# byungsook/deep-fluids

Measured on AMD Instinct MI355X. Metric: velocity-field voxels/sec (3D 64x96x64 train step), whole job; per-GPU in `per_gpu`, higher is better.
Workload: dtype f32; 1 GPU; cfg3: 3D smoke3 64x96x64 (Z,Y,X) fp32, GeneratorBE3 filters=128 num_conv=4, per-GPU batch 16, full train step (fwd+curl3+jacobian3+L1 losses+bwd+Adam); global_batch=16, batch_per_gpu=16, params=7483523, parallelism=dp1

## Files before the change

deep_fluids_amd/_lib.py:

```python
import ctypes
import os
import re

_HERE = os.path.dirname(os.path.abspath(__file__))
LIB_PATH = os.path.join(_HERE, "csrc", "libdeepfluids_hip.so")
TUNING_LIB_PATH = os.path.join(_HERE, "csrc", "libdeepfluids_hip_tuning.so")
HEADER_PATH = os.path.join(os.path.dirname(_HERE), "include", "deepfluids_hip.h")

P, I64, I32, F32 = ctypes.c_void_p, ctypes.c_int64, ctypes.c_int, ctypes.c_float

SIGNATURES = {
    "df_version": (I32, []),
    "df_last_error": (ctypes.c_char_p, []),
    "df_curl2d_fwd": (I32, [P, P, I64, I64, I64, P]),
    "df_curl2d_bwd": (I32, [P, P, I64, I64, I64, P]),
    "df_jacobian2d_fwd": (I32, [P, P, P, I64, I64, I64, P]),
    "df_jacobian2d_bwd": (I32, [P, P, P, I64, I64, I64, P]),
    "df_jacobian3d_fwd": (I32, [P, P, P, I64, I64, I64, I64, P]),
    "df_jacobian3d_bwd": (I32, [P, P, P, I64, I64, I64, I64, P]),
    "df_divergence2d": (I32, [P, P, I64, I64, I64, P]),
    "df_divergence3d": (I32, [P, P, I64, I64, I64, I64, P]),
    "df_velocity_loss3d_workspace_bytes": (I64, [I64, I64, I64, I64]),
    "df_velocity_loss3d_fwd": (I32, [P, P, P, P, P, I64, I64, I64, I64, P, I64, P]),
    "df_velocity_loss3d_bwd": (I32, [P, P, P, P, P, I64, I64, I64, I64, P, I64, P]),
# ... 21 lines not shown
    "df_concat2_fwd": (I32, [P, P, P, I64, I64, I64, P]),
    "df_concat2_bwd": (I32, [P, P, P, I64, I64, I64, P]),
    "df_dilate2_odd": (I32, [P, P, I64, I64, I64, I64, I64, I32, P]),
    "df_kl_bernoulli_fwd": (I32, [P, I64, I64, I64, F32, P, P]),
    "df_kl_bernoulli_bwd": (I32, [P, P, F32, P, I64, I64, I64, F32, P]),
    "df_sigmoid_fwd": (I32, [P, P, I64, P]),
    "df_sigmoid_bwd": (I32, [P, P, P, I64, P]),
    "df_mse_mean_fwd": (I32, [P, P, I64, P, P, I64, P]),
    "df_mse_mean_bwd": (I32, [P, P, P, F32, P, I64, P]),
    "df_colsum_workspace_bytes": (I64, [I64, I64]),
    "df_colsum": (I32, [P, P, I64, I64, P, I64, P]),
    "df_adam_tf1_step": (I32, [P, P, P, P, I64, F32, F32, F32, F32, F32, P]),
    "df_conv_packed_elems": (I64, [I64, I64, I64, I32]),
    "df_conv_pack_weights": (I32, [P, P, I64, I64, I64, I32, P]),
    "df_conv_fwd": (I32, [P, P, P, P, P, P, I64, I64, I64, I64, I64, I64, I32, I32, F32, P]),
    "df_conv_s2_fwd": (I32, [P, P, P, P, I64, I64, I64, I64, I64, I64, I32, I32, F32, P]),
    "df_conv_s2_wgrad_workspace_bytes": (I64, [I64, I64, I64, I64, I64, I64, I32]),
    "df_conv_s2_wgrad": (I32, [P, P, P, P, I64, I64, I64, I64, I64, I64, I32, P, I64, P]),
    "df_conv_s2_dgrad": (I32, [P, P, P, I64, I64, I64, I64, I64, I64, I32, P]),
    "df_conv_s2_dgrad_form": (I32, [P, I64, I64]),
    "df_upconv_packed_elems": (I64, [I64, I64, I32, I32]),
    "df_upconv_pack_weights": (I32, [P, P, I64, I64, I32, I32, P]),
    "df_upconv_fwd": (I32, [P, P, P, P, I64, I64, I64, I64, I64, I64, I32, I32, F32, P]),
    "df_upconv_dgrad": (I32, [P, P, P, I64, I64, I64, I64, I64, I64, I32, P]),
    "df_upconv_wgrad_workspace_bytes": (I64, [I64, I64, I64, I64, I64, I64, I32]),
    "df_upconv_wgrad": (I32, [P, P, P, P, I64, I64, I64, I64, I64, I64, I32, P, I64, P]),
    "df_add_up2x": (I32, [P, P, P, I64, I64, I64, I64, I64, I32, P]),
    "df_wino_packed_elems": (I64, [I64, I64, I32]),
    "df_wino_pack_weights": (I32, [P, P, I64, I64, I32, P]),
    "df_wino_conv_fwd": (I32, [P, P, P, P, P, P, I64, I64, I64, I64, I64, I64, I32, F32, P]),
    "df_wino_conv_fwd_addup": (I32, [P, P, P, P, P, P, I64, I64, I64, I64, I64, I64, F32, P]),
    "df_wino_conv_fwd_addup_bits": (I32, [P, P, P, P, P, P, I64, I64, I64, I64, I64, I64, F32, P]),
    "df_lrelu_bits_bwd_pool2x": (I32, [P, P, P, P, F32, I64, I64, I64, I64, I64, P]),
    "df_wino_upconv_fwd": (I32, [P, P, P, P, I64, I64, I64, I64, I64, I64, I32, F32, P]),
    "df_wino_upconv_dgrad": (I32, [P, P, P, I64, I64, I64, I64, I64, I64, P]),
    "df_wino_signbits_bytes": (I64, [I64, I64, I64, I64, I64]),
    "df_wino_conv_fwd_bits": (I32, [P, P, P, P, P, P, I64, I64, I64, I64, I64, I64, I32, F32, P]),
    "df_wino_upconv_fwd_bits": (I32, [P, P, P, P, P, I64, I64, I64, I64, I64, I64, F32, P]),
    "df_wino43_packed_elems": (I64, [I64, I64, I32]),
    "df_wino43_pack_weights": (I32, [P, P, I64, I64, I32, P]),
    "df_wino43_conv": (I32, [P, P, P, P, P, P, P, P, P, I64, I64, I64, I64, I64, I64, I32, F32, P]),
    "df_wino2d43_packed_elems": (I64, [I64, I64, I32]),
    "df_wino2d43_pack_weights": (I32, [P, P, I64, I64, I32, P]),
    "df_wino2d43_conv": (I32, [P, P, P, P, P, P, I64, I64, I64, I64, I64, I32, F32, P]),
    "df_wino2d43_signbits_bytes": (I64, [I64, I64, I64, I64]),
    "df_wino2d43_conv_bits": (I32, [P, P, P, P, P, P, I64, I64, I64, I64, I64, I32, F32, P]),
    "df_wino2d43_conv_addup_bits": (I32, [P, P, P, P, P, P, I64, I64, I64, I64, I64, F32, P]),
    "df_lrelu_words2d_bwd_pool2x": (I32, [P, P, P, P, F32, I64, I64, I64, I64, P]),
    "df_wino2d_packed_elems": (I64, [I64, I64, I32]),
    "df_wino2d_pack_weights": (I32, [P, P, I64, I64, I32, P]),
    "df_wino2d_conv_fwd": (I32, [P, P, P, P, P, P, I64, I64, I64, I64, I64, I32, F32, P]),
    "df_wino2d_upconv_fwd": (I32, [P, P, P, P, I64, I64, I64, I64, I64, I32, F32, P]),
    "df_wino2d_upconv_dgrad": (I32, [P, P, P, I64, I64, I64, I64, I64, P]),
    "df_conv_packed_elems_bf16x3": (I64, [I64, I64, I64, I32]),
    "df_conv_pack_weights_bf16x3": (I32, [P, P, I64, I64, I64, I32, P]),
    "df_conv_fwd_bf16x3": (I32, [P, P, P, P, P, P, I64, I64, I64, I64, I64, I64, I32, I32, F32, P]),
    "df_upconv_packed_elems_bf16x3": (I64, [I64, I64, I32, I32]),
    "df_upconv_pack_weights_bf16x3": (I32, [P, P, I64, I64, I32, I32, P]),
    "df_upconv_fwd_bf16x3": (I32, [P, P, P, P, I64, I64, I64, I64, I64, I64, I32, I32, F32, P]),
    "df_upconv_dgrad_bf16x3": (I32, [P, P, P, I64, I64, I64, I64, I64, I64, I32, P]),
    "df_conv_wgrad_bf16x3": (I32, [P, P, P, P, I64, I64, I64, I64, I64, I64, I32, P, I64, P]),
    "df_upconv_wgrad_bf16x3": (I32, [P, P, P, P, I64, I64, I64, I64, I64, I64, I32, P, I64, P]),
    "df_adam_tf1_step_dev": (I32, [P, P, P, P, I64, P, F32, F32, F32, P]),
    "df_gd_step": (I32, [P, P, I64, F32, F32, P]),
    "df_gd_step_dev": (I32, [P, P, I64, P, P]),
    "df_store_scalars": (I32, [P, I64, F32, F32, F32, F32, P]),
# ... 164 lines not shown
```

deep_fluids_amd/csrc/conv_small.hip:

```cpp
#include "conv_args.hpp"

namespace dfconv {
namespace {

using df::ceil_div;
typedef float f32x2 __attribute__((ext_vector_type(2)));

template <int KZ, int TZ, int TY, int TX, int CO, bool VEC>
__global__ __launch_bounds__(kThreads) void conv_small_n_kernel(const ConvArgs a) {
  static_assert(TZ * TY * TX == kThreads, "one thread per output voxel");
  constexpr int PZ = KZ / 2;
  constexpr int HZ = TZ + KZ - 1, HY = TY + 2, HX = TX + 2, HV = HZ * HY * HX;
  constexpr int NPIECE = HV * (CK / 4);
  constexpr int NLOAD = (NPIECE + kThreads - 1) / kThreads;
  constexpr int NTAP = KZ * 9;
  constexpr int S4 = LDS_STRIDE / 4;
  __shared__ __attribute__((aligned(16))) float sA[HV * LDS_STRIDE];
  __shared__ __attribute__((aligned(16))) f32x4 sWt[NTAP * 4 * 4];
  const f32x4* sA4 = reinterpret_cast<const f32x4*>(sA);

  const int tid = threadIdx.x;
  const int tile = xcd_tile(blockIdx.x, a.ntiles);
  const int ix = tile % a.nx;
  int t2 = tile / a.nx;
// ... 342 lines not shown
  t.RS = a.W * a.Cin + 8;
  const size_t lds = static_cast<size_t>(4) * 19 * t.RS * sizeof(float);
  const int wps = a.Cout == 128 ? 2 : 1;
  int ns = 4 / wps * df::kCUs;
  if (ns > t.nrows) ns = t.nrows / 2 * 2;
  t.rows_per = (t.nrows + ns - 1) / ns;
  t.flags = a.flags; t.leak = a.leak;
  dim3 grid((unsigned)ceil_div(ceil_div(t.nrows, t.rows_per) * wps, 4));
  const bool two = a.W * a.Cin > 256;
#define DF_TK2(CI, COV, NPV)                                                                                                                \
  do {                                                                                                                                      \
    if (lds > 64 * 1024)                                                                                                                    \
      if (hipError_t e = hipFuncSetAttribute(reinterpret_cast<const void*>(&conv_thin_k_mfma_kernel<CI, COV, NPV>),                         \
                                             hipFuncAttributeMaxDynamicSharedMemorySize, (int)lds))                                         \
        return df::fail((int)e, "df_conv_fwd(thin-K mfma): dynamic LDS opt-in: %s", hipGetErrorString(e));                                  \
    hipLaunchKernelGGL((conv_thin_k_mfma_kernel<CI, COV, NPV>), grid, dim3(kThreads), lds, s, t);                                           \
  } while (0)
#define DF_TK(CI)                                                                                                                           \
  do {                                                                                                                                      \
    if (a.Cout == 128) { if (two) DF_TK2(CI, 128, 2); else DF_TK2(CI, 128, 1); }                                                            \
    else { if (two) DF_TK2(CI, 64, 2); else DF_TK2(CI, 64, 1); }                                                                            \
  } while (0)
  switch (a.Cin) {
    case 1: DF_TK(1); break;
    case 2: DF_TK(2); break;
    case 3: DF_TK(3); break;
    default: DF_TK(4); break;
  }
#undef DF_TK
#undef DF_TK2
  return df::launched("df_conv_fwd(thin-K mfma)");
}

struct ThinNArgs {
  const float* x;
  const f32x4* wp;
  const float* bias;
  float* y;
  int B, D, H, W;
  int K8, Npad;
  int nsplit, rows_per;
  int flags;
  float leak;
};

template <int CO, int CIN>
__global__ __launch_bounds__(kThreads, 1) void conv_thin_n_mfma_kernel(const ThinNArgs a) {
  constexpr int NC = 9 * CO;
  constexpr int QN = CIN / 8;
  constexpr int NIT = 3 * QN;
  extern __shared__ __attribute__((aligned(16))) float smem_thin_n[];
  const int lane = threadIdx.x & 63;
  const int wave = __builtin_amdgcn_readfirstlane(threadIdx.x >> 6);
  const int stream = xcd_tile(blockIdx.x, gridDim.x) * 4 + wave;
  const int W = a.W, H = a.H, RS = W * CO + 8;
  float* ring = smem_thin_n + wave * 3 * RS;
  const int plane = stream / a.nsplit, part = stream % a.nsplit;
  if (plane >= a.B * a.D) return;
  const int y0 = part * a.rows_per;
  int y1 = y0 + a.rows_per;
  if (y1 > H) y1 = H;
  if (y0 >= y1) return;
  const int z = plane % a.D, b = plane / a.D;
  for (int i = lane; i < 3 * RS; i += 64) ring[i] = 0.f;
  const int n = lane & 31, kk = lane >> 5;

// ... 136 lines not shown
    default: DF_TN(3); break;
  }
#undef DF_TN
  return df::launched("df_conv_fwd(thin-N mfma)");
}

template <int KZ, int TZ, int TY, int TX>
int launch_small_k_t(ConvArgs a, hipStream_t s) {
  a.nz = (int)ceil_div(a.D, TZ); a.ny = (int)ceil_div(a.H, TY); a.nx = (int)ceil_div(a.W, TX);
  const int64_t nt = static_cast<int64_t>(a.B) * a.nz * a.ny * a.nx;
  DF_REQUIRE(nt < (1LL << 31), DF_ESHAPE, "df_conv_fwd: too many tiles");
  a.ntiles = (int)nt;
  const int nwn = a.Cout > 128 ? 4 : (a.Cout > 64 ? 2 : 1);
  dim3 grid((unsigned)nt, (unsigned)ceil_div(a.Cout, nwn * 64));
  hipLaunchKernelGGL((conv_small_k_kernel<KZ, TZ, TY, TX>), grid, dim3(kThreads), 0, s, a, nwn);
  return df::launched("df_conv_fwd(small-K)");
}

}

int launch_small_n(const ConvArgs& a, int kz, hipStream_t s) {
  if (thin_n_mfma_ok(a, kz) && !(a.flags & DF_CONV_VALU_ONLY)) return launch_thin_n_mfma(a, s);
  if (kz == 3) return a.W >= 12 ? launch_small_n_t<3, 4, 4, 16>(a, s) : launch_small_n_t<3, 4, 8, 8>(a, s);
  return a.W >= 12 ? launch_small_n_t<1, 1, 16, 16>(a, s) : launch_small_n_t<1, 1, 32, 8>(a, s);
}

int launch_small_k(const ConvArgs& a, int kz, hipStream_t s) {
  if (thin_k_mfma_ok(a, kz) && !(a.flags & DF_CONV_VALU_ONLY)) return launch_thin_k_mfma(a, s);
  if (kz == 3) return a.W >= 12 ? launch_small_k_t<3, 2, 4, 16>(a, s) : launch_small_k_t<3, 4, 4, 8>(a, s);
  return a.W >= 12 ? launch_small_k_t<1, 1, 8, 16>(a, s) : launch_small_k_t<1, 1, 16, 8>(a, s);
}

}
```

deep_fluids_amd/ops.py:

```python
import contextlib
import contextlib as _contextlib
import math
import os as _os
import threading as _threading

import numpy as np
import torch

from . import _lib
from ._lib import call, query, DF_CONV_BIAS, DF_CONV_LRELU, DF_CONV_MASK, DF_CONV_RESIDUAL

__all__ = [
    "lrelu", "conv2d", "conv3d", "linear", "upscale", "upscale3", "resize_nearest_neighbor", "reshape",
    "int_shape", "get_conv_shape", "nchw_to_nhwc", "nhwc_to_nchw", "add", "concat", "sigmoid", "mse_mean",
    "jacobian", "jacobian3", "curl", "curl3", "divergence", "divergence3", "pgrad",
    "vort_np", "curl_np", "grad_np", "jacobian_np3", "l1_mean", "velocity_loss",
    "denorm_img", "plane_view", "denorm_img3", "plane_view_np", "velocity_views3", "add_channels", "remove_channels",
    "advect", "advect_sequence", "advect_workspace", "density_image", "sphere_mask",
    "advect_velocity", "wall_buoyancy", "solve_pressure", "pressure_workspace", "smoke_step", "simulate_smoke", "default_buoyancy_force", "default_max_iter", "obstacle_flags", "ObstacleFlags",
    "open_sides", "SphereSource",
    "advect_particles", "particle_cells", "particle_levelset", "liquid_sequence", "seed_particles", "box_levelset", "sphere_levelset",
    "variable_scope", "get_variables", "get_variable", "reset_variables", "set_random_seed", "all_variables",
]

# ... 315 lines not shown
    if algo == 3 and WINO3D_FAMILY == "f224":
        call("df_wino43_conv", _ptr(x), _ptr(wp), _ptr(bias), _ptr(residual), _ptr(mask_src), _ptr(mask_bits), _ptr(y), None, _ptr(sign_bits),
             B, D, H, W, cin, cout, flags, float(leak), _stream())
        return y
    if algo == 3:
        if sign_bits is not None or mask_bits is not None:
            call("df_wino_conv_fwd_bits", _ptr(x), _ptr(wp), _ptr(bias), _ptr(mask_bits), _ptr(y), _ptr(sign_bits), B, D, H, W, cin, cout,
                 flags, float(leak), _stream())
            return y
        call("df_wino_conv_fwd", _ptr(x), _ptr(wp), _ptr(bias), _ptr(residual), _ptr(mask_src), _ptr(y), B, D, H, W, cin, cout,
             flags, float(leak), _stream())
        return y
    if (sign_bits is not None or mask_bits is not None) and not (algo == 2 and _w2fam(mode) == "f24"):
        raise _lib.DeepFluidsHipError("sign-bit masks exist for the 3-D Winograd kernels and the 2-D F(2,3) x F(4,3) kernel only")
    if algo == 2 and _w2fam(mode) == "f24" and (sign_bits is not None or mask_bits is not None):
        call("df_wino2d43_conv_bits", _ptr(x), _ptr(wp), _ptr(bias), _ptr(mask_bits), _ptr(y), _ptr(sign_bits), B, H, W, cin, cout, flags, float(leak),
             _stream())
        return y
    if algo == 2 and _w2fam(mode) == "f24":
        call("df_wino2d43_conv", _ptr(x), _ptr(wp), _ptr(bias), _ptr(residual), _ptr(mask_src), _ptr(y), B, H, W, cin, cout, flags, float(leak),
             _stream())
        return y
    if algo == 2:
        call("df_wino2d_conv_fwd", _ptr(x), _ptr(wp), _ptr(bias), _ptr(residual), _ptr(mask_src), _ptr(y), B, H, W, cin, cout,
             flags, float(leak), _stream())
        return y
    if THIN_VALU_ONLY:
        flags |= _lib.DF_CONV_VALU_ONLY
    call("df_conv_fwd" + _sfx(cin, cout), _ptr(x), _ptr(wp), _ptr(bias), _ptr(residual), _ptr(mask_src), _ptr(y), B, D, H, W,
         cin, cout, kz, flags, float(leak), _stream())
    return y


class _ConvSame3(torch.autograd.Function):

    @staticmethod
    def forward(ctx, x, w, b, leak):
        x = _prep(x, "x"); w = _prep(w, "weights"); b = _prep(b, "biases")
        nd = x.dim() - 2
        kz = 3 if nd == 3 else 1
        taps = 27 if nd == 3 else 9
        cin, cout = w.shape[-2], w.shape[-1]
        if tuple(w.shape[:-2]) != (3,) * nd or x.shape[-1] != cin:
            raise ValueError("conv: weights %s do not match input %s (k=3 only)" % (tuple(w.shape), tuple(x.shape)))
        dims = (x.shape[0], x.shape[1] if nd == 3 else 1, x.shape[-3], x.shape[-2])
        wp = _pack(w, taps, cin, cout, 0, dims)
        flags = DF_CONV_BIAS | (DF_CONV_LRELU if leak is not None else 0)
        y = _conv_raw(x, wp, b, None, None, dims, cin, cout, kz, flags, leak if leak is not None else 0.0)
        y = y.view(x.shape[:-1] + (cout,))
        if ACTIVATION_FETCH is not None and leak is not None:
            ACTIVATION_FETCH.append(y)
        ctx.save_for_backward(x, w, y if leak is not None else None)
        ctx.leak = leak
        ctx.geom = (dims, cin, cout, kz, taps)
        ctx.bptr = b.data_ptr()
        return y

    @staticmethod
    def backward(ctx, gy):
        x, w, y = ctx.saved_tensors
        dims, cin, cout, kz, taps = ctx.geom
        B, D, H, W = dims
        gy = _prep(gy, "grad")
        if ctx.leak is not None:
            dp = torch.empty_like(gy)
            call("df_lrelu_bwd", _ptr(gy), _ptr(y), _ptr(dp), float(ctx.leak), gy.numel(), _stream())
        else:
            dp = gy
        gw, rw = _grad_out(w.data_ptr(), w.shape, x.device)
        gb, rb = _grad_out(ctx.bptr, (cout,), x.device)
        _wgrad(x, dp, gw, gb, B, D, H, W, cin, cout, kz, _sfx(cin, cout))
        gx = None
        if ctx.needs_input_grad[0]:
            wpd = _pack(w, taps, cin, cout, 1, dims)
            gx = _conv_raw(dp, wpd, None, None, None, dims, cout, cin, kz, 0, 0.0).view(x.shape)
        return gx, rw, rb, None


class _GenBlock(torch.autograd.Function):

    @staticmethod
    def forward(ctx, x0, leak, *wb):
        x0 = _prep(x0, "x")
        n = len(wb) // 2
        nd = x0.dim() - 2
        kz = 3 if nd == 3 else 1
        taps = 27 if nd == 3 else 9
        dims = (x0.shape[0], x0.shape[1] if nd == 3 else 1, x0.shape[-3], x0.shape[-2])
        xs = [x0]
        bits = []
        x = x0
        for i in range(n):
            w = _prep(wb[2 * i], "weights"); b = _prep(wb[2 * i + 1], "biases")
            cin, cout = w.shape[-2], w.shape[-1]
            if tuple(w.shape[:-2]) != (3,) * nd or x.shape[-1] != cin:
                raise ValueError("gen_block: weights %s do not match input %s" % (tuple(w.shape), tuple(x.shape)))
            wp = _pack(w, taps, cin, cout, 0, dims)
            bk = _bits_kind(cin, cout, dims, kz) if i < n - 1 else 0
            sb = _new_bits(dims, cout, x0, bk) if bk else None
            bits.append(sb)
            x = _conv_raw(x, wp, b, None, None, dims, cin, cout, kz, DF_CONV_BIAS | DF_CONV_LRELU, leak, sign_bits=sb).view(
                x0.shape[:-1] + (cout,))
            xs.append(x)
        if x.shape != x0.shape:
            raise ValueError("gen_block: residual add needs Cout == Cin of the block")
        y = torch.empty_like(x)
        call("df_add", _ptr(x), _ptr(x0), _ptr(y), x.numel(), _stream())
        if ACTIVATION_FETCH is not None:
# ... 165 lines not shown
                    if SIGN_BITS_FETCH is not None:
                        SIGN_BITS_FETCH.append((tail_bits, fdims, cout))
                    x = None
                elif i == n - 1 and is3d and _use_wino(cin, cout, fdims, kz) == 3:
                    f224 = WINO3D_FAMILY == "f224"
                    _count("conv", "winograd-%s+addup" % ("f2x2x4" if f224 else "f2x2x2"), fdims, cin, cout)
                    x_in, x = x, torch.empty(fshape, dtype=torch.float32, device=xc.device)
                    y = torch.empty(fshape, dtype=torch.float32, device=xc.device)
                    if f224:
                        call("df_wino43_conv", _ptr(x_in), _ptr(wp), _ptr(b), _ptr(xc), None, None, _ptr(x), _ptr(y), None, fdims[0], fdims[1],
                             fdims[2], fdims[3], cin, cout, DF_CONV_BIAS | DF_CONV_LRELU | _lib.DF_CONV_ADDUP, float(leak), _stream())
                    else:
                        call("df_wino_conv_fwd_addup", _ptr(x_in), _ptr(wp), _ptr(b), _ptr(xc), _ptr(x), _ptr(y), fdims[0], fdims[1],
                             fdims[2], fdims[3], cin, cout, float(leak), _stream())
                elif i == n - 1 and not is3d and _bits_kind(cin, cout, fdims, kz) == 2 and ACTIVATION_FETCH is None:
                    _count("conv", "winograd-f2x4+addup+signwords", fdims, cin, cout)
                    tail_bits = _new_bits(fdims, cout, xc, 2)
                    y = torch.empty(fshape, dtype=torch.float32, device=xc.device)
                    call("df_wino2d43_conv_addup_bits", _ptr(x), _ptr(wp), _ptr(b), _ptr(xc), _ptr(y), _ptr(tail_bits), fdims[0], fdims[2], fdims[3], cin, cout,
                         float(leak), _stream())
                    x = None
                else:
                    x = _conv_raw(x, wp, b, None, None, fdims, cin, cout, kz, DF_CONV_BIAS | DF_CONV_LRELU, leak, sign_bits=sb).view(fshape)
            xs.append(x)
        if y is None:
            y = torch.empty_like(x)
            call("df_add_up2x", _ptr(x), _ptr(xc), _ptr(y), cdims[0], cdims[1], cdims[2], cdims[3], C, int(is3d), _stream())
        if ACTIVATION_FETCH is not None:
            ACTIVATION_FETCH.extend(xs)
        ctx.save_for_backward(*([xc] + xs + [wb[2 * i] for i in range(n)]))
        ctx.geom = (n, cdims, fdims, kz, taps, float(leak), C, is3d)
        ctx.bits = bits
        ctx.tail_bits = tail_bits
        ctx.bptrs = [wb[2 * i + 1].data_ptr() for i in range(n)]
        return y

    @staticmethod
    def backward(ctx, dy):
        n, cdims, fdims, kz, taps, leak, C, is3d = ctx.geom
        saved = ctx.saved_tensors
        xc, xs, ws = saved[0], saved[1:n + 1], saved[n + 1:]
        B, D, H, W = fdims
        dy = _prep(dy, "grad")
        dp = torch.empty_like(dy)
        dxc = None
        if ctx.tail_bits is not None:
            dxc = torch.empty_like(xc)
            if is3d:
                call("df_lrelu_bits_bwd_pool2x", _ptr(dy), _ptr(ctx.tail_bits), _ptr(dp), _ptr(dxc), leak, cdims[0], cdims[1], cdims[2], cdims[3],
                     C, _stream())
            else:
                call("df_lrelu_words2d_bwd_pool2x", _ptr(dy), _ptr(ctx.tail_bits), _ptr(dp), _ptr(dxc), leak, cdims[0], cdims[2], cdims[3], C, _stream())
        elif ctx.needs_input_grad[0]:
            dxc = torch.empty_like(xc)
            call("df_lrelu_bwd_pool2x", _ptr(dy), _ptr(xs[n - 1]), _ptr(dp), _ptr(dxc), leak, cdims[0], cdims[1], cdims[2], cdims[3], C,
                 int(is3d), _stream())
        else:
            call("df_lrelu_bwd", _ptr(dy), _ptr(xs[n - 1]), _ptr(dp), leak, dy.numel(), _stream())
        grads = [None] * (2 * n)
        lane = _WgradLane(fdims, dy, taps)
        for i in range(n, 0, -1):
            w = ws[i - 1]
            gw, rw = _grad_out(w.data_ptr(), w.shape, dy.device)
            gb, rb = _grad_out(ctx.bptrs[i - 1], (C,), dy.device)
            if i > 1:
                lane.run(lambda: _wgrad(xs[i - 2], dp, gw, gb, B, D, H, W, C, C, kz, _sfx(C, C)), dp, gw, gb)
                wpd = _pack(w, taps, C, C, 1, fdims)
                mb = ctx.bits[i - 2]
                dp = _conv_raw(dp, wpd, None, None, None if mb is not None else xs[i - 2], fdims, C, C, kz, DF_CONV_MASK, leak,
                               mask_bits=mb).view(dy.shape)
            else:
                nbytes = query("df_upconv_wgrad_workspace_bytes", cdims[0], cdims[1], cdims[2], cdims[3], C, C, kz)
                wsb = torch.empty((nbytes + 3) // 4, dtype=torch.float32, device=dy.device)

                def up_wgrad():
                    if _sfx(C, C):
                        call("df_upconv_wgrad" + _sfx(C, C), _ptr(xc), _ptr(dp), _ptr(gw), _ptr(gb), cdims[0], cdims[1], cdims[2],
                             cdims[3], C, C, kz, _ptr(wsb), nbytes, _stream())
                    else:
# ... 469 lines not shown


def lrelu(x, leak=0.2):
    return _Lrelu.apply(x, leak)


def add(a, b):
    return _Add.apply(a, b)


def concat(values, axis=-1):
    if len(values) != 2 or axis not in (-1, values[0].dim() - 1):
        raise NotImplementedError("concat: two tensors along the channel axis (the encoder's skip connection)")
    return _Concat2.apply(values[0], values[1])


def sigmoid(x):
    return _Sigmoid.apply(x)


def kl_bernoulli(z, n, rho):
    return _KlBernoulli.apply(z, n, rho)


def mse_mean(a, b):
    return _MseMean.apply(a, b)


FUSED_BLOCKS = True

ACTIVATION_FETCH = None


_OPTION_ATTRS = {"conv_precision": "CONV_PRECISION", "conv_algo": "CONV_ALGO", "wino3d_family": "WINO3D_FAMILY", "wino2d_family": "WINO2D_FAMILY", "wgrad_algo": "WGRAD_ALGO",
                 "thin_valu_only": "THIN_VALU_ONLY", "sign_bit_masks": "SIGN_BIT_MASKS", "fused_blocks": "FUSED_BLOCKS",
                 "dispatch_counts": "DISPATCH_COUNTS", "concurrent_wgrad_work": "CONCURRENT_WGRAD_WORK", "activation_fetch": "ACTIVATION_FETCH", "sign_bits_fetch": "SIGN_BITS_FETCH"}
_OPTION_CHOICES = {"conv_precision": ("fp32", "bf16x3"), "conv_algo": ("auto", "direct", "winograd"), "wino3d_family": ("f224", "f222"), "wino2d_family": ("auto", "f24", "f22"), "wgrad_algo": (0, 1, 2, 3, 4)}
_OPTION_LOCK = _threading.RLock()


@_contextlib.contextmanager
def options(**kw):
    for k, v in kw.items():
        if k not in _OPTION_ATTRS:
            raise TypeError("ops.options: unknown option %r (known: %s)" % (k, ", ".join(sorted(_OPTION_ATTRS))))
        if k in _OPTION_CHOICES and v not in _OPTION_CHOICES[k]:
            raise ValueError("ops.options: %s=%r not in %r" % (k, v, _OPTION_CHOICES[k]))
    g = globals()
    with _OPTION_LOCK:
        old = {k: g[_OPTION_ATTRS[k]] for k in kw}
        try:
            for k, v in kw.items():
                g[_OPTION_ATTRS[k]] = v
            yield
        finally:
            for k, v in old.items():
                g[_OPTION_ATTRS[k]] = v


def gen_block(x, filters, names, nd, leak=0.2):
    wb = []
    cin = int(x.shape[-1])
    for name in names:
        wb.append(get_variable(name + "/weights", (3,) * nd + (cin, int(filters)), "xavier", x.device))
        wb.append(get_variable(name + "/biases", (int(filters),), "zeros", x.device))
        cin = int(filters)
    return _GenBlock.apply(x, leak, *wb)
# ... 894 lines not shown
```

include/deepfluids_hip.h:

```cpp
#ifndef DEEPFLUIDS_HIP_H
#define DEEPFLUIDS_HIP_H

#include <stdint.h>

#ifdef __cplusplus
extern "C" {
#endif

#define DF_VERSION 207

enum {
  DF_OK = 0,
  DF_EINVAL = -1,
  DF_ESHAPE = -2,
  DF_EALIGN = -3,
  DF_EWORKSPACE = -4
};

enum {
  DF_CONV_LRELU = 1,
  DF_CONV_RESIDUAL = 2,
  DF_CONV_MASK = 4,
  DF_CONV_BIAS = 8,
  DF_CONV_ADDUP = 16,
// ... 145 lines not shown
int df_wino_upconv_dgrad(const float* g, const float* wp, float* acc, int64_t B, int64_t Dc, int64_t Hc, int64_t Wc, int64_t Cin,
                         int64_t Cout, df_stream_t stream);

int df_wino_conv_fwd_addup(const float* x, const float* wp, const float* bias, const float* xc, float* y, float* y2, int64_t B,
                           int64_t D, int64_t H, int64_t W, int64_t Cin, int64_t Cout, float leak, df_stream_t stream);

int64_t df_wino43_packed_elems(int64_t cin, int64_t cout, int mode);
int df_wino43_pack_weights(const float* w, float* wp, int64_t cin, int64_t cout, int mode, df_stream_t stream);
int df_wino43_conv(const float* x, const float* wp, const float* bias, const float* residual, const float* mask_src, const void* mask_bits,
                   float* y, float* y2, void* sign_bits, int64_t B, int64_t D, int64_t H, int64_t W, int64_t Cin, int64_t Cout, int flags,
                   float leak, df_stream_t stream);

int64_t df_wino2d43_packed_elems(int64_t cin, int64_t cout, int mode);
int df_wino2d43_pack_weights(const float* w, float* wp, int64_t cin, int64_t cout, int mode, df_stream_t stream);
int df_wino2d43_conv(const float* x, const float* wp, const float* bias, const float* residual, const float* mask_src, float* y, int64_t B,
                     int64_t H, int64_t W, int64_t Cin, int64_t Cout, int flags, float leak, df_stream_t stream);
int64_t df_wino2d43_signbits_bytes(int64_t B, int64_t H, int64_t W, int64_t C);
int df_wino2d43_conv_bits(const float* x, const float* wp, const float* bias, const void* mask_bits, float* y, void* sign_bits, int64_t B, int64_t H,
                          int64_t W, int64_t Cin, int64_t Cout, int flags, float leak, df_stream_t stream);
int df_wino2d43_conv_addup_bits(const float* x, const float* wp, const float* bias, const float* xc, float* y2, void* sign_bits, int64_t B, int64_t H,
                                int64_t W, int64_t Cin, int64_t Cout, float leak, df_stream_t stream);
int df_lrelu_words2d_bwd_pool2x(const float* gy, const void* mask_bits, float* gx, float* gpool, float leak, int64_t B, int64_t Hc, int64_t Wc, int64_t C,
                                df_stream_t stream);

int64_t df_wino_signbits_bytes(int64_t B, int64_t D, int64_t H, int64_t W, int64_t C);
int df_wino_conv_fwd_bits(const float* x, const float* wp, const float* bias, const void* mask_bits, float* y, void* sign_bits, int64_t B,
                          int64_t D, int64_t H, int64_t W, int64_t Cin, int64_t Cout, int flags, float leak, df_stream_t stream);
int df_wino_upconv_fwd_bits(const float* xc, const float* wp, const float* bias, float* y, void* sign_bits, int64_t B, int64_t Dc,
                            int64_t Hc, int64_t Wc, int64_t Cin, int64_t Cout, float leak, df_stream_t stream);
int df_wino_conv_fwd_addup_bits(const float* x, const float* wp, const float* bias, const float* xc, float* y2, void* sign_bits,
                                int64_t B, int64_t D, int64_t H, int64_t W, int64_t Cin, int64_t Cout, float leak, df_stream_t stream);
int df_lrelu_bits_bwd_pool2x(const float* gy, const void* mask_bits, float* gx, float* gpool, float leak, int64_t B, int64_t Dc, int64_t Hc,
                             int64_t Wc, int64_t C, df_stream_t stream);


int64_t df_wino2d_packed_elems(int64_t cin, int64_t cout, int mode);
int df_wino2d_pack_weights(const float* w, float* wp, int64_t cin, int64_t cout, int mode, df_stream_t stream);
int df_wino2d_conv_fwd(const float* x, const float* wp, const float* bias, const float* residual, const float* mask_src,
                       float* y, int64_t B, int64_t H, int64_t W, int64_t Cin, int64_t Cout, int flags, float leak,
                       df_stream_t stream);
int df_wino2d_upconv_fwd(const float* xc, const float* wp, const float* bias, float* y, int64_t B, int64_t Hc, int64_t Wc, int64_t Cin,
                         int64_t Cout, int flags, float leak, df_stream_t stream);
int df_wino2d_upconv_dgrad(const float* g, const float* wp, float* acc, int64_t B, int64_t Hc, int64_t Wc, int64_t Cin, int64_t Cout,
                           df_stream_t stream);


int64_t df_conv_packed_elems_bf16x3(int64_t taps, int64_t cin, int64_t cout, int mode);
int df_conv_pack_weights_bf16x3(const float* w, float* wp, int64_t taps, int64_t cin, int64_t cout, int mode,
                                df_stream_t stream);
int df_conv_fwd_bf16x3(const float* x, const float* wp, const float* bias, const float* residual, const float* mask_src,
                       float* y, int64_t B, int64_t D, int64_t H, int64_t W, int64_t Cin, int64_t Cout, int kz, int flags,
                       float leak, df_stream_t stream);
int64_t df_upconv_packed_elems_bf16x3(int64_t cin, int64_t cout, int kz, int mode);
int df_upconv_pack_weights_bf16x3(const float* w, float* wp, int64_t cin, int64_t cout, int kz, int mode,
                                  df_stream_t stream);
int df_upconv_fwd_bf16x3(const float* xc, const float* wp, const float* bias, float* y, int64_t B, int64_t Dc, int64_t Hc,
                         int64_t Wc, int64_t Cin, int64_t Cout, int kz, int flags, float leak, df_stream_t stream);
int df_upconv_dgrad_bf16x3(const float* g, const float* wp, float* acc, int64_t B, int64_t Dc, int64_t Hc, int64_t Wc,
                           int64_t Cin, int64_t Cout, int kz, df_stream_t stream);
int df_conv_wgrad_bf16x3(const float* x, const float* gy, float* gw, float* gb, int64_t B, int64_t D, int64_t H, int64_t W,
                         int64_t Cin, int64_t Cout, int kz, void* workspace, int64_t workspace_bytes, df_stream_t stream);
int df_upconv_wgrad_bf16x3(const float* xc, const float* gy, float* gw, float* gb, int64_t B, int64_t Dc, int64_t Hc,
                           int64_t Wc, int64_t Cin, int64_t Cout, int kz, void* workspace, int64_t workspace_bytes,
                           df_stream_t stream);

int64_t df_conv_wgrad_workspace_bytes(int64_t B, int64_t D, int64_t H, int64_t W, int64_t Cin, int64_t Cout, int kz);
// ... 130 lines not shown
```

Before: 35.55 million voxels/s.

## Fuse final thin conv dgrad with leaky-ReLU sign-bit backward and 2x pooling

Adds an MFMA kernel that computes the input-gradient of the final 128->3 conv and applies the leaky-ReLU sign-bit mask and 2x2x2 pooled upsample-gradient in the same pass. The conv backward hands its work to the preceding up-block through a zero stand-in gradient, so the full-resolution 128-channel gradient is never written and then re-read by a separate mask/pool kernel. The handoff depends on autograd ordering and on detecting the stand-in tensor by pointer and stride, and falls back to the unfused path when those checks fail.

Result: slower. 35.13 million voxels/s (-1.2%).

```diff
diff --git a/deep_fluids_amd/_lib.py b/deep_fluids_amd/_lib.py
--- a/deep_fluids_amd/_lib.py
+++ b/deep_fluids_amd/_lib.py
@@ -77,6 +77,8 @@
     "df_wino_conv_fwd_addup": (I32, [P, P, P, P, P, P, I64, I64, I64, I64, I64, I64, F32, P]),
     "df_wino_conv_fwd_addup_bits": (I32, [P, P, P, P, P, P, I64, I64, I64, I64, I64, I64, F32, P]),
     "df_lrelu_bits_bwd_pool2x": (I32, [P, P, P, P, F32, I64, I64, I64, I64, I64, P]),
+    "df_conv_thin_dgrad_bits_pool2x_ok": (I32, [I64, I64, I64, I64, I64, I64]),
+    "df_conv_thin_dgrad_bits_pool2x": (I32, [P, P, P, P, P, F32, I64, I64, I64, I64, I64, I64, P]),
     "df_wino_upconv_fwd": (I32, [P, P, P, P, I64, I64, I64, I64, I64, I64, I32, F32, P]),
     "df_wino_upconv_dgrad": (I32, [P, P, P, I64, I64, I64, I64, I64, I64, P]),
     "df_wino_signbits_bytes": (I64, [I64, I64, I64, I64, I64]),
diff --git a/deep_fluids_amd/csrc/conv_small.hip b/deep_fluids_amd/csrc/conv_small.hip
--- a/deep_fluids_amd/csrc/conv_small.hip
+++ b/deep_fluids_amd/csrc/conv_small.hip
@@ -398,6 +398,200 @@
   return df::launched("df_conv_fwd(thin-K mfma)");
 }
 
+constexpr int kBitBytesPerBlock = 1024;
+struct ThinKPoolArgs {
+  const float* g;
+  const f32x4* wp;
+  const unsigned char* bits;
+  float* gx;
+  float* gpool;
+  int Dc, Hc, W;
+  int tapstride;
+  int ncell, cells_per, RS;
+  int nbz, nby, nbx;
+  float leak;
+};
+
+template <int CI, int NCH>
+__global__ __launch_bounds__(kThreads, 1) void conv_thin_k_bits_pool_kernel(const ThinKPoolArgs a) {
+  constexpr int CO = 128, NK = 27 * CI, KS = (NK + 1) / 2, NP = NCH * 32 * CI > 256 ? 2 : 1;
+  extern __shared__ __attribute__((aligned(16))) float smem_thin_kp[];
+  const int lane = threadIdx.x & 63;
+  const int wave = __builtin_amdgcn_readfirstlane(threadIdx.x >> 6);
+  const int gwave = blockIdx.x * 4 + wave;
+  const int stream = gwave >> 1, half = gwave & 1;
+  const int RS = a.RS, W = a.W, WC = W * CI, D = 2 * a.Dc, H = 2 * a.Hc;
+  float* sG = smem_thin_kp + wave * 19 * RS;
+  const int c0 = stream * a.cells_per;
+  int c1 = c0 + a.cells_per;
+  if (c1 > a.ncell) c1 = a.ncell;
+  for (int i = lane; i < 19 * RS; i += 64) sG[i] = 0.f;
+  if (c0 >= c1) return;
+  const int kk = lane >> 5, n4 = half * 64 + (lane & 31) * 2;
+
+  float wr[KS][2];
+#pragma unroll
+  for (int s = 0; s < KS; ++s) {
+    const int k = 2 * s + kk;
+    const bool ok = k < NK;
+    const int tap = ok ? k / CI : 0, c = ok ? k % CI : 0;
+#pragma unroll
+    for (int j = 0; j < 2; ++j) {
+      const f32x4 rec = a.wp[static_cast<int64_t>(tap) * a.tapstride + n4 + j];
+      const float v = c == 0 ? rec[0] : c == 1 ? rec[1] : c == 2 ? rec[2] : rec[3];
+      wr[s][j] = ok ? v : 0.f;
+    }
+  }
+  const f32x2 bias2 = {0.f, 0.f};
+
+  const int nl4 = WC / 4;
+  f32x4 gq[NP][9];
+  auto load_g = [&](int it) {
+    const int cell = it >> 2;
+    const int yc = cell % a.Hc;
+    const int t = cell / a.Hc;
+    const int y = 2 * yc + (it & 1), z = 2 * (t % a.Dc) + ((it >> 1) & 1);
+    const int b = t / a.Dc;
+#pragma unroll
+    for (int k = 0; k < 9; ++k) {
+      const int zs = z + (k / 3 - 1), ys = y + (k % 3 - 1);
+      const bool ok = zs >= 0 && zs < D && ys >= 0 && ys < H;
+      const int zc = ok ? zs : z, yc2 = ok ? ys : y;
+      const float* src = a.g + ((static_cast<int64_t>(b) * D + zc) * H + yc2) * WC;
+#pragma unroll
+      for (int p = 0; p < NP; ++p) {
+        f32x4 v = {0.f, 0.f, 0.f, 0.f};
+        if (lane + 64 * p < nl4) v = *reinterpret_cast<const f32x4*>(src + (lane + 64 * p) * 4);
+        gq[p][k] = ok ? v : f32x4{0.f, 0.f, 0.f, 0.f};
+      }
+    }
+  };
+  auto store_g = [&](int buf) {
+#pragma unroll
+    for (int p = 0; p < NP; ++p)
+      if (lane + 64 * p < nl4) {
+#pragma unroll
+        for (int k = 0; k < 9; ++k) *reinterpret_cast<f32x4*>(sG + (buf * 9 + k) * RS + 4 + (lane + 64 * p) * 4) = gq[p][k];
+      }
+  };
+
+  const char* sGb = reinterpret_cast<const char*>(sG);
+  const int lanebase = (lane & 31) * CI * 4;
+  auto gather = [&](int buf, int x0, float (&av)[KS]) {
+    const int cb = lanebase + x0 * (CI * 4);
+    const int bb = buf * (9 * RS * 4);
+#pragma unroll
+    for (int s = 0; s < KS; ++s) {
+      const int k0 = 2 * s, k1 = 2 * s + 1;
+      const int o0 = ((k0 / CI / 3) * RS + 4 + ((k0 / CI) % 3 - 1) * CI + k0 % CI) * 4 + bb;
+      const int o1 = k1 < NK ? ((k1 / CI / 3) * RS + 4 + ((k1 / CI) % 3 - 1) * CI + k1 % CI) * 4 + bb : (18 * RS + 4) * 4;
+      av[s] = *reinterpret_cast<const float*>(sGb + cb + (kk ? o1 : o0));
+    }
+  };
+
+  const int Wc = W >> 1;
+  f32x2 pool[NCH][8];
+#pragma unroll
+  for (int c = 0; c < NCH; ++c)
+#pragma unroll
+    for (int q = 0; q < 8; ++q) pool[c][q] = f32x2{0.f, 0.f};
+  load_g(4 * c0);
+  store_g(0);
+  int buf = 0;
+  for (int it = 4 * c0; it < 4 * c1; ++it) {
+    const bool more = it + 1 < 4 * c1;
+    if (more) load_g(it + 1);
+    const int cell = it >> 2, rho = it & 3;
+    const int yc = cell % a.Hc;
+    const int t = cell / a.Hc;
+    const int zc = t % a.Dc, b = t / a.Dc;
+    const int64_t row = (static_cast<int64_t>(b) * D + (2 * zc + (rho >> 1))) * H + (2 * yc + (rho & 1));
+    const int64_t obase = row * W * CO + n4;
+    const unsigned char* brow = a.bits + ((static_cast<int64_t>(b) * a.nbz + (zc >> 1)) * a.nby + (yc >> 2)) * a.nbx * (4 * kBitBytesPerBlock) +
+                                ((n4 >> 5) * kBitBytesPerBlock + (zc & 1) * 512 + kk * 256 + ((n4 >> 4) & 1) * 64 + (yc & 3) * 16 + (n4 & 15));
+#pragma unroll
+    for (int chunk = 0; chunk < NCH; ++chunk) {
+      float av[KS];
+      gather(buf, chunk * 32, av);
+      const int64_t oc = obase + static_cast<int64_t>(chunk * 32) * CO;
+      unsigned mw[8];
+#pragma unroll
+      for (int q = 0; q < 8; ++q)
+        mw[q] = *reinterpret_cast<const unsigned short*>(brow + (chunk * 4 + (q >> 1)) * (4 * kBitBytesPerBlock) + (q & 1) * 128);
+      f32x16 acc[2];
+#pragma unroll
+      for (int j = 0; j < 2; ++j)
+#pragma unroll
+        for (int r = 0; r < 16; ++r) acc[j][r] = 0.f;
+#pragma unroll
+      for (int s = 0; s < KS; ++s)
+#pragma unroll
+        for (int j = 0; j < 2; ++j) acc[j] = __builtin_amdgcn_mfma_f32_32x32x2f32(av[s], wr[s][j], acc[j], 0, 0, 0);
+#pragma unroll
+      for (int r = 0; r < 16; ++r) {
+        const int q = 2 * (r >> 2) + ((r >> 1) & 1);
+        const f32x2 v = f32x2{acc[0][r], acc[1][r]} + bias2;
+        f32x2 p = pool[chunk][q];
+        if (rho == 0 && !(r & 1)) p = f32x2{0.f, 0.f};
+        pool[chunk][q] = p + v;
+        const unsigned m = mw[q] >> (2 * rho + (r & 1));
+        f32x2 o;
+        o[0] = (m & 1u) ? v[0] : a.leak * v[0];
+        o[1] = (m & 0x100u) ? v[1] : a.leak * v[1];
+        *reinterpret_cast<f32x2*>(a.gx + oc + ((r >> 2) * 8 + kk * 4 + (r & 3)) * CO) = o;
+      }
+      if (rho == 3) {
+        float* gp = a.gpool + (static_cast<int64_t>(cell) * Wc + chunk * 16 + kk * 2) * CO + n4;
+#pragma unroll
+        for (int q = 0; q < 8; ++q) *reinterpret_cast<f32x2*>(gp + ((q >> 1) * 4 + (q & 1)) * CO) = pool[chunk][q];
+      }
+      if (chunk == 0 && more) store_g(buf ^ 1);
+    }
+    buf ^= 1;
+  }
+}
+
+constexpr int kThinPoolCi = 3;
+
+inline bool thin_k_bits_pool_ok(int64_t B, int64_t D, int64_t H, int64_t W, int64_t Cin, int64_t Cout) {
+  return B > 0 && D > 0 && H > 0 && W > 0 && Cin == kThinPoolCi && Cout == 128 && D % 2 == 0 && H % 2 == 0 && W % 32 == 0 && W * Cin <= 448 &&
+         B * (D / 2) * (H / 2) < (1LL << 29) && 4 * 19 * (W * Cin + 8) * 4 <= df::lds_optin_bytes();
+}
+
+int launch_thin_k_bits_pool(const float* g, const float* wp, const void* bits, float* gx, float* gpool, float leak, int64_t B, int64_t D,
+                            int64_t H, int64_t W, hipStream_t s) {
+  constexpr int CI = kThinPoolCi;
+  ThinKPoolArgs t;
+  t.g = g; t.wp = reinterpret_cast<const f32x4*>(wp); t.bits = static_cast<const unsigned char*>(bits); t.gx = gx; t.gpool = gpool;
+  t.Dc = (int)(D / 2); t.Hc = (int)(H / 2); t.W = (int)W;
+  t.tapstride = 2 * 2 * 128;
+  t.ncell = (int)(B * t.Dc * t.Hc);
+  t.RS = (int)W * CI + 8;
+  t.nbz = (int)ceil_div(D, 4); t.nby = (int)ceil_div(H, 8); t.nbx = (int)ceil_div(W, 8);
+  t.leak = leak;
+  const size_t lds = static_cast<size_t>(4) * 19 * t.RS * sizeof(float);
+  int ns = 2 * df::kCUs;
+  if (ns > t.ncell) ns = t.ncell;
+  t.cells_per = (t.ncell + ns - 1) / ns;
+  dim3 grid((unsigned)ceil_div(ceil_div(t.ncell, t.cells_per) * 2, 4));
+#define DF_TKP(NCHV)                                                                                                                        \
+  do {                                                                                                                                      \
+    if (lds > 64 * 1024)                                                                                                                    \
+      if (hipError_t e = hipFuncSetAttribute(reinterpret_cast<const void*>(&conv_thin_k_bits_pool_kernel<CI, NCHV>),                        \
+                                             hipFuncAttributeMaxDynamicSharedMemorySize, (int)lds))                                         \
+        return df::fail((int)e, "df_conv_thin_dgrad_bits_pool2x: dynamic LDS opt-in: %s", hipGetErrorString(e));                            \
+    hipLaunchKernelGGL((conv_thin_k_bits_pool_kernel<CI, NCHV>), grid, dim3(kThreads), lds, s, t);                                          \
+  } while (0)
+  switch (W / 32) {
+    case 1: DF_TKP(1); break;
+    case 2: DF_TKP(2); break;
+    case 3: DF_TKP(3); break;
+    default: DF_TKP(4); break;
+  }
+#undef DF_TKP
+  return df::launched("df_conv_thin_dgrad_bits_pool2x");
+}
+
 struct ThinNArgs {
   const float* x;
   const f32x4* wp;
@@ -600,3 +794,23 @@
 }
 
 }
+
+extern "C" {
+
+int df_conv_thin_dgrad_bits_pool2x_ok(int64_t B, int64_t D, int64_t H, int64_t W, int64_t Cin, int64_t Cout) {
+  return dfconv::thin_k_bits_pool_ok(B, D, H, W, Cin, Cout) ? 1 : 0;
+}
+
+int df_conv_thin_dgrad_bits_pool2x(const float* gy, const float* wp, const void* mask_bits, float* gx, float* gpool, float leak, int64_t B,
+                                   int64_t D, int64_t H, int64_t W, int64_t Cin, int64_t Cout, df_stream_t stream) {
+  DF_REQUIRE(gy && wp && mask_bits && gx && gpool, DF_EINVAL, "df_conv_thin_dgrad_bits_pool2x: null pointer");
+  DF_REQUIRE(B > 0 && D > 0 && H > 0 && W > 0 && Cin > 0 && Cout > 0, DF_EINVAL, "df_conv_thin_dgrad_bits_pool2x: non-positive extent");
+  DF_REQUIRE(dfconv::thin_k_bits_pool_ok(B, D, H, W, Cin, Cout), DF_ESHAPE,
+             "df_conv_thin_dgrad_bits_pool2x: only 3 -> 128 channels, even D and H, W a multiple of 32 up to 128 "
+             "(elsewhere: df_conv_fwd + df_lrelu_bits_bwd_pool2x)");
+  DF_REQUIRE(df::aligned16(gy) && df::aligned16(wp) && df::aligned16(mask_bits) && df::aligned16(gx) && df::aligned16(gpool), DF_EALIGN,
+             "df_conv_thin_dgrad_bits_pool2x: 16-byte alignment");
+  return dfconv::launch_thin_k_bits_pool(gy, wp, mask_bits, gx, gpool, leak, B, D, H, W, df::as_stream(stream));
+}
+
+}
diff --git a/deep_fluids_amd/ops.py b/deep_fluids_amd/ops.py
--- a/deep_fluids_amd/ops.py
+++ b/deep_fluids_amd/ops.py
@@ -371,6 +371,17 @@
     return y
 
 
+THIN_TAIL_FUSED = _os.environ.get("DF_THIN_TAIL_FUSED", "1") != "0"
+
+
+def _thin_tail_src(x, leak, dims, cin, cout, kz):
+    src = x.grad_fn
+    if (not THIN_TAIL_FUSED or THIN_VALU_ONLY or leak is not None or kz != 3 or getattr(src, "_forward_cls", None) is not _UpGenBlock
+            or getattr(src, "tail_bits", None) is None):
+        return None
+    return src if query("df_conv_thin_dgrad_bits_pool2x_ok", dims[0], dims[1], dims[2], dims[3], cout, cin) == 1 else None
+
+
 class _ConvSame3(torch.autograd.Function):
 
     @staticmethod
@@ -393,6 +404,7 @@
         ctx.leak = leak
         ctx.geom = (dims, cin, cout, kz, taps)
         ctx.bptr = b.data_ptr()
+        ctx.tail_src = _thin_tail_src(x, leak, dims, cin, cout, kz)
         return y
 
     @staticmethod
@@ -412,7 +424,11 @@
         gx = None
         if ctx.needs_input_grad[0]:
             wpd = _pack(w, taps, cin, cout, 1, dims)
-            gx = _conv_raw(dp, wpd, None, None, None, dims, cout, cin, kz, 0, 0.0).view(x.shape)
+            if ctx.tail_src is not None:
+                gx = torch.zeros(1, dtype=torch.float32, device=x.device).expand(x.shape)
+                ctx.tail_src.thin_tail = (dp, wpd, cout, gx)
+            else:
+                gx = _conv_raw(dp, wpd, None, None, None, dims, cout, cin, kz, 0, 0.0).view(x.shape)
         return gx, rw, rb, None
 
 
@@ -644,6 +660,7 @@
         ctx.geom = (n, cdims, fdims, kz, taps, float(leak), C, is3d)
         ctx.bits = bits
         ctx.tail_bits = tail_bits
+        ctx.thin_tail = None
         ctx.bptrs = [wb[2 * i + 1].data_ptr() for i in range(n)]
         return y
 
@@ -653,10 +670,26 @@
         saved = ctx.saved_tensors
         xc, xs, ws = saved[0], saved[1:n + 1], saved[n + 1:]
         B, D, H, W = fdims
-        dy = _prep(dy, "grad")
-        dp = torch.empty_like(dy)
+        tail, ctx.thin_tail = ctx.thin_tail, None
         dxc = None
-        if ctx.tail_bits is not None:
+        fused_tail = False
+        if tail is not None:
+            g, wpt, cg, standin = tail
+            if dy.data_ptr() == standin.data_ptr() and not any(dy.stride()):
+                fused_tail = True
+                _count("conv", "thin+tail-signwords", fdims, cg, C)
+                dp = torch.empty(dy.shape, dtype=torch.float32, device=dy.device)
+                dxc = torch.empty_like(xc)
+                call("df_conv_thin_dgrad_bits_pool2x", _ptr(g), _ptr(wpt), _ptr(ctx.tail_bits), _ptr(dp), _ptr(dxc), leak, B, D, H, W, cg, C,
+                     _stream())
+            else:
+                dy = _prep(dy, "grad") + _conv_raw(g, wpt, None, None, None, fdims, cg, C, kz, 0, 0.0).view(dy.shape)
+        if not fused_tail:
+            dy = _prep(dy, "grad")
+            dp = torch.empty_like(dy)
+        if fused_tail:
+            pass
+        elif ctx.tail_bits is not None:
             dxc = torch.empty_like(xc)
             if is3d:
                 call("df_lrelu_bits_bwd_pool2x", _ptr(dy), _ptr(ctx.tail_bits), _ptr(dp), _ptr(dxc), leak, cdims[0], cdims[1], cdims[2], cdims[3],
@@ -1192,7 +1225,7 @@
 ACTIVATION_FETCH = None
 
 
-_OPTION_ATTRS = {"conv_precision": "CONV_PRECISION", "conv_algo": "CONV_ALGO", "wino3d_family": "WINO3D_FAMILY", "wino2d_family": "WINO2D_FAMILY", "wgrad_algo": "WGRAD_ALGO",
+_OPTION_ATTRS = {"thin_tail_fused": "THIN_TAIL_FUSED", "conv_precision": "CONV_PRECISION", "conv_algo": "CONV_ALGO", "wino3d_family": "WINO3D_FAMILY", "wino2d_family": "WINO2D_FAMILY", "wgrad_algo": "WGRAD_ALGO",
                  "thin_valu_only": "THIN_VALU_ONLY", "sign_bit_masks": "SIGN_BIT_MASKS", "fused_blocks": "FUSED_BLOCKS",
                  "dispatch_counts": "DISPATCH_COUNTS", "concurrent_wgrad_work": "CONCURRENT_WGRAD_WORK", "activation_fetch": "ACTIVATION_FETCH", "sign_bits_fetch": "SIGN_BITS_FETCH"}
 _OPTION_CHOICES = {"conv_precision": ("fp32", "bf16x3"), "conv_algo": ("auto", "direct", "winograd"), "wino3d_family": ("f224", "f222"), "wino2d_family": ("auto", "f24", "f22"), "wgrad_algo": (0, 1, 2, 3, 4)}
diff --git a/include/deepfluids_hip.h b/include/deepfluids_hip.h
--- a/include/deepfluids_hip.h
+++ b/include/deepfluids_hip.h
@@ -201,6 +201,9 @@
                                 int64_t B, int64_t D, int64_t H, int64_t W, int64_t Cin, int64_t Cout, float leak, df_stream_t stream);
 int df_lrelu_bits_bwd_pool2x(const float* gy, const void* mask_bits, float* gx, float* gpool, float leak, int64_t B, int64_t Dc, int64_t Hc,
                              int64_t Wc, int64_t C, df_stream_t stream);
+int df_conv_thin_dgrad_bits_pool2x_ok(int64_t B, int64_t D, int64_t H, int64_t W, int64_t Cin, int64_t Cout);
+int df_conv_thin_dgrad_bits_pool2x(const float* gy, const float* wp, const void* mask_bits, float* gx, float* gpool, float leak, int64_t B,
+                                   int64_t D, int64_t H, int64_t W, int64_t Cin, int64_t Cout, df_stream_t stream);
 
 
 int64_t df_wino2d_packed_elems(int64_t cin, int64_t cout, int mode);
```
